# hardcamls/video-coding

Hardware: AMD Instinct MI355X
Metric: Mpixel/s decoded (1080p 4:2:0 batch) (higher is better)
Workload: dtype int32

## Files before the change

### video-coding_amd/csrc/hvc_capi.hip

```cpp
#include <cmath>

#include "hvc_ctx.h"
#include "hvc_dct_fixed.h"

bool pin_to_ctx_cpus(const hvc_ctx *c) {
    if (!c->have_cpus) {
        if (c->have_default_cpus) (void)pthread_setaffinity_np(pthread_self(), sizeof(cpu_set_t), &c->default_cpus);
        return true;
    }
    return pthread_setaffinity_np(pthread_self(), sizeof(cpu_set_t), &c->cpus) == 0;
}

bool parse_cpulist(const char *s, cpu_set_t &set) {
    CPU_ZERO(&set);
    int n = 0;
    while (*s) {
        while (*s == ' ' || *s == '\n') s++;
        if (!*s) break;
        char *end = nullptr;
        const long a = std::strtol(s, &end, 10);
        if (end == s || a < 0) return false;
        long b = a;
        s = end;
        if (*s == '-') {
// ... 147 lines not shown
    bool ok = g.ok && hipStreamCreateWithFlags(&c->own_stream, hipStreamNonBlocking) == hipSuccess &&
              hipEventCreate(&c->ev0) == hipSuccess && hipEventCreate(&c->ev1) == hipSuccess &&
              [&] {
                  for (int i = 0; i < HVC_PROF_RING; i++)
                      if (hipEventCreate(&c->k0[i]) != hipSuccess || hipEventCreate(&c->k1[i]) != hipSuccess) return false;
                  return true;
              }() &&
              hipMalloc((void **)&c->d_fix_count, HVC_FIX_WORDS * sizeof(unsigned)) == hipSuccess &&
              hipMemset(c->d_fix_count, 0, HVC_FIX_WORDS * sizeof(unsigned)) == hipSuccess;
    if (!ok) {
        hvc_destroy(c);
        return HVC_E_NO_DEVICE;
    }
    c->stream = c->own_stream;
    c->have_default_cpus = sched_getaffinity(0, sizeof c->default_cpus, &c->default_cpus) == 0;
    if (const char *env = std::getenv("HVC_HOST_CPUS")) (void)hvc_set_host_cpus(c, env);
    *out = c;
    return HVC_OK;
} HVC_ABI_CATCH

void hvc_destroy(hvc_ctx *c) {
    if (!c) return;
    c->pool.shutdown();
    DeviceGuard g(c->device);
    (void)hipStreamSynchronize(c->stream);
    if (c->own_stream) (void)hipStreamSynchronize(c->own_stream);
    if (c->copy_stream) (void)hipStreamSynchronize(c->copy_stream);
    if (c->down_stream) (void)hipStreamSynchronize(c->down_stream);
    if (c->side_stream) (void)hipStreamSynchronize(c->side_stream);
    for (int i = 0; i < 3; i++)
        if (c->rd_stream[i]) (void)hipStreamSynchronize(c->rd_stream[i]);
    if (c->d_fix_count) (void)hipFree(c->d_fix_count);
    if (c->d_fix_list) (void)hipFree(c->d_fix_list);
    if (c->d_in) (void)hipFree(c->d_in);
    if (c->d_out) (void)hipFree(c->d_out);
    if (c->d_div_px) (void)hipFree(c->d_div_px);
    if (c->d_div_in) (void)hipFree(c->d_div_in);
    if (c->d_div_out) (void)hipFree(c->d_div_out);
    if (c->d_dct_tab) (void)hipFree(c->d_dct_tab);
    if (c->d_dct_a) (void)hipFree(c->d_dct_a);
    if (c->d_dct_b) (void)hipFree(c->d_dct_b);
    if (c->d_sums) (void)hipFree(c->d_sums);
    if (c->d_aux) (void)hipFree(c->d_aux);
    if (c->d_aux2) (void)hipFree(c->d_aux2);
    if (c->ev0) (void)hipEventDestroy(c->ev0);
    if (c->ev1) (void)hipEventDestroy(c->ev1);
    for (int i = 0; i < HVC_PROF_RING; i++) {
        if (c->k0[i]) (void)hipEventDestroy(c->k0[i]);
        if (c->k1[i]) (void)hipEventDestroy(c->k1[i]);
    }
    for (int i = 0; i < hvc_ctx::RING; i++) {
        if (c->h_ring[i]) (void)hipHostFree(c->h_ring[i]);
        if (c->d_ring[i]) (void)hipFree(c->d_ring[i]);
        if (c->d_oring[i]) (void)hipFree(c->d_oring[i]);
        if (c->ev_h2d[i]) (void)hipEventDestroy(c->ev_h2d[i]);
        if (c->ev_kern[i]) (void)hipEventDestroy(c->ev_kern[i]);
        if (c->eh_in[i]) (void)hipHostFree(c->eh_in[i]);
        if (c->eh_out[i]) (void)hipHostFree(c->eh_out[i]);
        if (c->ed_in[i]) (void)hipFree(c->ed_in[i]);
        if (c->ed_out[i]) (void)hipFree(c->ed_out[i]);
        if (c->ev_up[i]) (void)hipEventDestroy(c->ev_up[i]);
        if (c->ev_down[i]) (void)hipEventDestroy(c->ev_down[i]);
        for (int k = 0; k < 3; k++)
            if (c->ev_et[i][k]) (void)hipEventDestroy(c->ev_et[i][k]);
        if (c->ev_gpu[i]) (void)hipEventDestroy(c->ev_gpu[i]);
        if (c->gp_h_ecs[i]) (void)hipHostFree(c->gp_h_ecs[i]);
// ... 269 lines not shown
    return HVC_OK;
} HVC_ABI_CATCH

int hvc_checksum_records(hvc_ctx *c, const void *data, size_t record_bytes, size_t record_stride, int n_records,
                         uint64_t *sums, int where) try {
    if (!c || !sums || n_records < 0 || (!data && n_records && record_bytes)) return HVC_E_INVALID_ARG;
    if (where != HVC_MEM_HOST && where != HVC_MEM_DEVICE) return HVC_E_INVALID_ARG;
    if (n_records == 0) return HVC_OK;
    if (n_records > 1 && record_stride < record_bytes) return HVC_E_INVALID_ARG;
    DeviceGuard g(c->device);
    if (!g.ok) return fail_hip(c, hipErrorInvalidDevice);
    const size_t sum_bytes = (size_t)n_records * sizeof(unsigned long long);
    const uint8_t *d = (const uint8_t *)data;
    int r;
    if (where == HVC_MEM_HOST) {
        const size_t bytes = (size_t)(n_records - 1) * record_stride + record_bytes;
        if ((r = grow(c, &c->d_in, &c->in_cap, bytes ? bytes : 1))) return r;
        if (bytes) HIPCHK(c, hipMemcpyAsync(c->d_in, data, bytes, hipMemcpyHostToDevice, c->stream));
        d = (const uint8_t *)c->d_in;
    }
    if ((r = grow(c, &c->d_sums, &c->sums_cap, sum_bytes))) return r;
    for (int r0 = 0; r0 < n_records; r0 += 65535)
        HIPCHK(c, hvc::launch_checksum(d + (size_t)r0 * record_stride, record_bytes, record_stride,
                                       n_records - r0 < 65535 ? n_records - r0 : 65535, (unsigned long long *)c->d_sums + r0, c->stream));
    HIPCHK(c, hipMemcpyAsync(sums, c->d_sums, sum_bytes, hipMemcpyDeviceToHost, c->stream));
    HIPCHK(c, hipStreamSynchronize(c->stream));
    return HVC_OK;
} HVC_ABI_CATCH

int hvc_last_wide_blocks(hvc_ctx *c, uint64_t *count) try {
    if (!c || !count) return HVC_E_INVALID_ARG;
    DeviceGuard g(c->device);
    unsigned long long v = 0;
    HIPCHK(c, hipMemcpyAsync(&v, c->d_fix_count + 2, sizeof v, hipMemcpyDeviceToHost, c->stream));
    HIPCHK(c, hipStreamSynchronize(c->stream));
    *count = c->wide_host >= 0 ? (uint64_t)c->wide_host : (uint64_t)v;
    return HVC_OK;
} HVC_ABI_CATCH

static void prepare_tables(const uint16_t *qtabs, int n_qtabs, int *qt, int *ethr, int *ethr_packed, unsigned *qpair) {
    for (int i = 0; i < n_qtabs * 64; i++) qt[i] = (int)qtabs[i];
    for (int t = 0; t < n_qtabs; t++) {
        unsigned qmax = 1;
        for (int i = 0; i < 64; i++) qmax = qtabs[t * 64 + i] > qmax ? qtabs[t * 64 + i] : qmax;
        unsigned long long m = HVC_GUARD_D / qmax;
        unsigned long long thr = m * m;
        ethr[t] = thr > 0x7ffffffeull ? 0x7ffffffe : (int)thr;
        m = HVC_GUARD_D_PACKED / qmax;
        thr = m * m;
        ethr_packed[t] = thr > 0x7ffffffeull ? 0x7ffffffe : (int)thr;
        static const int PAIRS[4][2] = {{HVC_PAIR_A_LO, HVC_PAIR_A_HI}, {HVC_PAIR_B_LO, HVC_PAIR_B_HI},
                                        {HVC_PAIR_C_LO, HVC_PAIR_C_HI}, {HVC_PAIR_Z_LO, HVC_PAIR_Z_HI}};
        for (int r = 0; r < 8; r++)
            for (int k = 0; k < 4; k++) {
                unsigned lo = qtabs[t * 64 + hvc::HVC_ZF[8 * r + PAIRS[k][0]]];
                unsigned hi = qtabs[t * 64 + hvc::HVC_ZF[8 * r + PAIRS[k][1]]];
                qpair[t * 32 + r * 4 + k] = (lo & 0xffffu) | (hi << 16);
            }
    }
}

static int upload_dcfix(hvc_ctx *c, const std::vector<unsigned> &ids, const std::vector<long long> &dcs, const unsigned **d_count,
                        const unsigned **d_ids, const long long **d_dcs) {
    const size_t n = ids.size();
    const size_t off_ids = 16, off_dcs = (off_ids + n * sizeof(unsigned) + 15) & ~(size_t)15;
    int r = grow(c, &c->d_dcfix, &c->dcfix_cap, off_dcs + n * sizeof(long long));
    if (r) return r;
// ... 173 lines not shown
    int per = frames_per_launch(n_frames, blocks_per_frame);
    if (per > 65535) per = 65535;
    const unsigned long long by_ids = ids_per_frame ? ((1ull << 32) - 1) / ids_per_frame : (unsigned long long)per;
    if ((unsigned long long)per > by_ids) per = (int)by_ids;
    return per < 1 ? 1 : per;
}

int decode_frames_impl(hvc_ctx *c, const int16_t *coefs, size_t coef_fs, const uint16_t *qtabs, int n_qtabs,
                       const hvc_component *comps_in, int n_comp_in, int n_frames, uint8_t *pixels, size_t pixel_fs, int where,
                       const int16_t *dc_plane, size_t dc_fs, const std::vector<WideFix> *wide) {
    if (!c || n_frames < 0) return HVC_E_INVALID_ARG;
    if (where != HVC_MEM_HOST && where != HVC_MEM_DEVICE) return HVC_E_INVALID_ARG;
    int r = check_qtabs(qtabs, n_qtabs, false);
    if (r) return r;
    hvc_component kept[HVC_MAX_COMP];
    int n_comp = 0;
    if ((r = drop_empty_components(comps_in, n_comp_in, kept, &n_comp))) return r;
    if (n_comp == 0) return HVC_OK;
    const hvc_component *const comps = kept;
    if (!coefs || !pixels) return HVC_E_INVALID_ARG;
    Layout L;
    r = make_layout(comps, n_comp, n_qtabs, L);
    if (r) return r;
    if (n_frames == 0) return HVC_OK;
    if (n_frames > 1 && (coef_fs < L.coef_span || pixel_fs < L.pixel_span)) return HVC_E_INVALID_ARG;
    if ((coef_fs & 7) || (pixel_fs & 7)) return HVC_E_ALIGNMENT;
    const unsigned long long ids_per_frame = (unsigned long long)L.tiles_per_frame * HVC_TILE;
    const int per = frames_per_launch_capped(n_frames, L.blocks_per_frame, ids_per_frame);
    if (wide && !wide->empty() && (unsigned long long)n_frames * ids_per_frame >= (1ull << 32)) return HVC_E_TOO_LARGE;
    DeviceGuard g(c->device);
    if (!g.ok) return fail_hip(c, hipErrorInvalidDevice);

    const bool twin = c->arith == HVC_ARITH_HARDCAML;
    size_t need = twin ? 0 : (size_t)((unsigned long long)per * ids_per_frame);
    if (need > c->fix_cap) {
        void *p = c->d_fix_list;
        size_t cap = c->fix_cap * sizeof(unsigned);
        r = grow(c, &p, &cap, need * sizeof(unsigned));
        c->d_fix_list = (unsigned *)p;
        c->fix_cap = cap / sizeof(unsigned);
        if (r) return r;
    }

    hvc::DecodeParams P;
    std::memset(&P, 0, sizeof P);
    P.coef_fs = coef_fs;
    P.pixel_fs = pixel_fs;
    P.n_frames = n_frames;
    P.n_comp = L.n_comp;
    P.tiles_per_frame = L.tiles_per_frame;
    for (int i = 0; i < L.n_comp; i++) P.comp[i] = L.comp[i];
    prepare_tables(qtabs, n_qtabs, P.qt, P.ethr, P.ethr_packed, P.qpair);
    wide_total_begin(c);
    fix_assign(c, P);

    bool wide_only = false;
    for (int i = 0; i < n_qtabs * 64; i++) wide_only |= qtabs[i] > 255;
    wide_only |= c->decode_kernel == 2;
    P.kernel_sel = (c->decode_kernel == 1 || c->decode_kernel == 3) ? c->decode_kernel : 0;
    if (wide_only) c->wide_host = (long long)((unsigned long long)n_frames * L.blocks_per_frame);
    if (twin) c->wide_host = 0;
    auto launch = [&](hvc::DecodeParams &Q, hipEvent_t k0, hipEvent_t k1) -> hipError_t {
        if (twin) return hvc::launch_hardcaml(hardcaml_params(Q, qtabs, n_qtabs), c->stream, k0, k1);
        if (wide_only) return hvc::launch_decode_wide_only(Q, c->stream, k0, k1);
        fix_assign(c, Q);
        const hipError_t e = hvc::launch_decode(Q, c->stream, k0, k1);
        if (e == hipSuccess) fix_commit(c);
        else fix_reset(c);
        return e;
    };
    auto launch_range = [&](const int16_t *d_coefs, uint8_t *d_pixels, int f0, int cnt, hipEvent_t k0, hipEvent_t k1) -> hipError_t {
        for (int f = f0; f < f0 + cnt; f += per) {
            hvc::DecodeParams Pk = P;
            Pk.n_frames = f0 + cnt - f < per ? f0 + cnt - f : per;
            Pk.coefs = d_coefs + (size_t)f * coef_fs;
            Pk.pixels = d_pixels + (size_t)f * pixel_fs;
            if (dc_plane) Pk.dc_plane = dc_plane + (size_t)f * dc_fs;
            const hipError_t e = launch(Pk, f == f0 ? k0 : nullptr, f + per >= f0 + cnt ? k1 : nullptr);
            if (e != hipSuccess) return e;
        }
        return hipSuccess;
    };

    if (where == HVC_MEM_DEVICE) {
        if (((uintptr_t)coefs & 15) || ((uintptr_t)pixels & 7)) return HVC_E_ALIGNMENT;
        if (dc_plane && P.kernel_sel != 0 && !twin) return HVC_E_INVALID_ARG;
        P.coefs = coefs;
        P.pixels = pixels;
        P.dc_plane = dc_plane;
        P.dc_fs = dc_fs;
        const bool prof = c->profiling;
        const int slot = (int)(c->k_calls % HVC_PROF_RING);
        HIPCHK(c, launch_range(coefs, pixels, 0, n_frames, prof ? c->k0[slot] : nullptr, prof ? c->k1[slot] : nullptr));
        if (prof) c->k_calls++;
        if (wide && !wide->empty()) return apply_wide_dc(c, P, *wide, qtabs, n_qtabs);
        return HVC_OK;
    }
    if (dc_plane || (wide && !wide->empty())) return HVC_E_INVALID_ARG;

    size_t cbytes = ((size_t)(n_frames - 1) * coef_fs + L.coef_span) * sizeof(int16_t);
    size_t pbytes = (size_t)(n_frames - 1) * pixel_fs + L.pixel_span;
// ... 217 lines not shown
    const bool aligned = width % 16 == 0 && frame_stride % 16 == 0 && (where == HVC_MEM_HOST || (uintptr_t)frames % 16 == 0);
    hvc::plan_decode_444(P, aligned);
    const unsigned long long ids_per_frame = (unsigned long long)P.tiles_per_frame * HVC_TILE * P.nw;
    const int per = frames_per_launch_capped(n_frames, L.blocks_per_frame, ids_per_frame);
    if (wide && !wide->empty() && (unsigned long long)n_frames * ids_per_frame >= (1ull << 32)) return HVC_E_TOO_LARGE;
    const unsigned long long ids = (unsigned long long)per * ids_per_frame;
    DeviceGuard g(c->device);
    if (!g.ok) return fail_hip(c, hipErrorInvalidDevice);
    if ((size_t)ids > c->fix_cap) {
        void *p = c->d_fix_list;
        size_t cap = c->fix_cap * sizeof(unsigned);
        r = grow(c, &p, &cap, (size_t)ids * sizeof(unsigned));
        c->d_fix_list = (unsigned *)p;
        c->fix_cap = cap / sizeof(unsigned);
        if (r) return r;
    }
    int ethr_unused[HVC_MAX_QTABS];
    prepare_tables(qtabs, n_qtabs, P.qt, ethr_unused, P.ethr_packed, P.qpair);
    bool wide_only = c->decode_kernel == 2;
    for (int i = 0; i < n_qtabs * 64; i++) wide_only |= qtabs[i] > 255;
    P.fix_list = c->d_fix_list;
    wide_total_begin(c);
    const int split = (aligned && !wide_only && c->decode_kernel == 0 && height % 8 == 0 && P.pl[0].cbw == P.pl[0].bw) ? fused444_mode() : 0;
    const size_t luma_ids = split ? (size_t)per * (size_t)((P.pl[0].cbw * P.pl[0].cbh + HVC_TILE - 1) / HVC_TILE) * HVC_TILE : 0;
    if (luma_ids + (size_t)ids > c->fix_cap) {
        void *p = c->d_fix_list;
        size_t cap = c->fix_cap * sizeof(unsigned);
        r = grow(c, &p, &cap, (luma_ids + (size_t)ids) * sizeof(unsigned));
        c->d_fix_list = (unsigned *)p;
        c->fix_cap = cap / sizeof(unsigned);
        if (r) return r;
        P.fix_list = c->d_fix_list;
    }
    if (split == 2 && !c->side_stream) {
        static const int prio_sel = [] { const char *v = std::getenv("HVC_444_SIDE_PRIO"); return v ? std::atoi(v) : 0; }();
        int least = 0, greatest = 0;
        HIPCHK(c, hipDeviceGetStreamPriorityRange(&least, &greatest));
        HIPCHK(c, hipStreamCreateWithPriority(&c->side_stream, hipStreamNonBlocking, prio_sel < 0 ? greatest : prio_sel > 0 ? least : 0));
        HIPCHK(c, hipEventCreateWithFlags(&c->ev_fork, hipEventDisableTiming));
        HIPCHK(c, hipEventCreateWithFlags(&c->ev_join, hipEventDisableTiming));
    }
    auto launch_split = [&](hvc::Decode444Params &Q, hipEvent_t k0, hipEvent_t k1) -> hipError_t {
        const hvc::Plane444K &K = Q.pl[0];
        hvc::DecodeParams Y;
        std::memset(&Y, 0, sizeof Y);
        Y.coefs = Q.coefs;
        Y.pixels = Q.out;
        Y.coef_fs = Q.coef_fs;
        Y.pixel_fs = Q.out_fs;
        Y.n_frames = Q.n_frames;
        Y.n_comp = 1;
        Y.comp[0].bw = K.cbw;
        Y.comp[0].bh = K.cbh;
        Y.comp[0].nblk = K.cbw * K.cbh;
        Y.comp[0].magic = K.cbw == 1 ? 0u : (unsigned)(((1ull << 32) + (unsigned)K.cbw - 1) / (unsigned)K.cbw);
        Y.comp[0].qtab = K.qtab;
        Y.comp[0].coef_off = K.coef_off;
        Y.comp[0].plane_off = K.out_off;
        Y.comp[0].stride = (size_t)Q.width;
        Y.tiles_per_frame = (Y.comp[0].nblk + HVC_TILE - 1) / HVC_TILE;
        prepare_tables(qtabs, n_qtabs, Y.qt, Y.ethr, Y.ethr_packed, Y.qpair);
        Y.dc_plane = Q.dc_plane;
        Y.dc_fs = Q.dc_fs;
        Y.fix_count = c->d_fix_count + 4 + c->fix_phase_l;
        Y.fix_count_next = c->d_fix_count + 4 + (c->fix_phase_l ^ 1);
        Y.fix_list = c->d_fix_list + (size_t)ids;
        Y.wide_total = reinterpret_cast<unsigned long long *>(c->d_fix_count + 2);
        fix_assign(c, Q);
        Q.tile0 = Q.y_tiles;
        hipStream_t ys = c->stream;
        hipError_t e = hipSuccess;
        if (k0) e = hipEventRecord(k0, c->stream);
        if (split == 2) {
            if (e == hipSuccess && !c->wide_total_started) e = hipMemsetAsync(Y.wide_total, 0, sizeof(unsigned long long), c->stream);
            Y.wide_first = Q.wide_first = 2;
            if (e == hipSuccess) e = hipEventRecord(c->ev_fork, c->stream);
            if (e == hipSuccess) e = hipStreamWaitEvent(c->side_stream, c->ev_fork, 0);
            ys = c->side_stream;
        } else {
            Y.wide_first = Q.wide_first;
            Q.wide_first = 0;
        }
        if (e == hipSuccess) e = hvc::launch_decode(Y, ys, nullptr, nullptr);
        if (e == hipSuccess) c->fix_phase_l ^= 1;
        if (e == hipSuccess) e = hvc::launch_decode_444(Q, false, c->stream, nullptr, nullptr);
        if (e == hipSuccess && split == 2) {
            e = hipEventRecord(c->ev_join, c->side_stream);
            if (e == hipSuccess) e = hipStreamWaitEvent(c->stream, c->ev_join, 0);
        }
        if (e == hipSuccess && k1) e = hipEventRecord(k1, c->stream);
        if (e == hipSuccess) fix_commit(c);
        else {
            if (c->side_stream) (void)hipStreamSynchronize(c->side_stream);
            fix_reset(c);
        }
        return e;
    };
    auto launch = [&](hvc::Decode444Params &Q, hipEvent_t k0, hipEvent_t k1) -> hipError_t {
        if (wide_only) {
            c->wide_host = (long long)n_frames * ((long long)P.pl[0].cbw * P.pl[0].cbh + 2ll * P.pl[1].cbw * P.pl[1].cbh);
            return hvc::launch_decode_444(Q, true, c->stream, k0, k1);
        }
        if (split) return launch_split(Q, k0, k1);
        fix_assign(c, Q);
        const hipError_t e = hvc::launch_decode_444(Q, false, c->stream, k0, k1);
        if (e == hipSuccess) fix_commit(c);
        else fix_reset(c);
        return e;
    };

    auto launch_range = [&](const int16_t *d_coefs, uint8_t *d_out, int f0, int cnt, hipEvent_t k0, hipEvent_t k1) -> hipError_t {
        for (int f = f0; f < f0 + cnt; f += per) {
            hvc::Decode444Params Pk = P;
            Pk.n_frames = f0 + cnt - f < per ? f0 + cnt - f : per;
            Pk.coefs = d_coefs + (size_t)f * coef_fs;
            Pk.out = d_out + (size_t)f * frame_stride;
            if (dc_plane) Pk.dc_plane = dc_plane + (size_t)f * dc_fs;
// ... 594 lines not shown
```

### video-coding_amd/csrc/hvc_ctx.h

```cpp
#ifndef HVC_CTX_H
#define HVC_CTX_H

#include <hip/hip_runtime.h>
#include <pthread.h>
#include <sched.h>

#include <algorithm>
#include <atomic>
#include <chrono>
#include <condition_variable>
#include <cstdio>
#include <cstdlib>
#include <cstring>
#include <mutex>
#include <new>
#include <thread>
#include <deque>
#include <functional>
#include <vector>

#include "../../include/hvc_jpeg.h"
#include "hvc_hdec.h"
#include "hvc_hardcaml.h"
#include "hvc_huff.h"
#include "hvc_kernels.h"
#include "hvc_pool.h"

#define HVC_PROF_RING 64
#define HVC_FIX_WORDS 8

struct hvc_ctx {
    int device = -1;
    hipStream_t own_stream = nullptr;
    hipStream_t stream = nullptr;
    hipEvent_t ev0 = nullptr, ev1 = nullptr;
    hipEvent_t k0[HVC_PROF_RING] = {}, k1[HVC_PROF_RING] = {};
    unsigned long long k_calls = 0;
    bool profiling = false;
    bool honour_restart = false;
    int decode_kernel = 0;
    int arith = HVC_ARITH_MODEL;
    int enc_arith = HVC_ARITH_MODEL;
    int huff_tables = HVC_HUFF_DEFAULT;
    int restart_interval = 0;
    unsigned *d_fix_count = nullptr;
    int fix_phase_l = 0;
    hipStream_t side_stream = nullptr;
    hipEvent_t ev_fork = nullptr, ev_join = nullptr;
    bool wide_total_started = false;
    long long wide_host = -1;
    int fix_phase = 0;
    int fix_last = 0;
    unsigned *d_fix_list = nullptr;
    size_t fix_cap = 0;
    void *d_in = nullptr, *d_out = nullptr, *d_sums = nullptr, *d_aux = nullptr, *d_aux2 = nullptr;
    size_t in_cap = 0, out_cap = 0, sums_cap = 0, aux_cap = 0, aux2_cap = 0;
    void *d_div_px = nullptr, *d_div_in = nullptr, *d_div_out = nullptr;
    size_t div_px_cap = 0, div_in_cap = 0, div_out_cap = 0;
    void *d_dct_tab = nullptr, *d_dct_a = nullptr, *d_dct_b = nullptr;
    size_t dct_a_cap = 0, dct_b_cap = 0;
    int last_hip = 0;
    static constexpr int RING = 3;
    hipStream_t copy_stream = nullptr, down_stream = nullptr;
    hipStream_t rd_stream[3] = {};
    hipEvent_t ev_rd[3] = {};
    void *h_ring[RING] = {}, *d_ring[RING] = {}, *d_oring[RING] = {};
    size_t ring_bytes = 0, oring_bytes = 0;
    hipEvent_t ev_h2d[RING] = {}, ev_kern[RING] = {}, ev_t[4] = {};
    void *eh_in[RING] = {}, *ed_in[RING] = {}, *eh_out[RING] = {}, *ed_out[RING] = {};
    size_t e_in_bytes = 0, e_out_bytes = 0;
    hipEvent_t ev_up[RING] = {}, ev_down[RING] = {}, ev_et[RING][3] = {}, ev_gpu[RING] = {};
    void *ed_seg[RING] = {}, *ed_off[RING] = {}, *eh_off[RING] = {};
    size_t e_seg_bytes = 0, e_off_bytes = 0;
    void *eh_specs[RING] = {};
    size_t e_specs_bytes = 0;
    void *gp_h_ecs[RING] = {}, *gp_d_ecs[RING] = {}, *gp_h_meta[RING] = {}, *gp_d_meta[RING] = {};
    void *gp_h_ftabs[RING] = {}, *gp_d_ftabs[RING] = {};
    size_t gp_ecs_bytes = 0, gp_meta_bytes = 0, gp_ftabs_bytes = 0;
    void *gd_ecs = nullptr, *gd_meta = nullptr, *gd_state = nullptr, *gd_tables = nullptr, *gd_coefs = nullptr, *gd_dcd = nullptr;
    void *gd_h_ecs = nullptr;
    size_t gd_h_ecs_cap = 0;
    void *gd_fcnt = nullptr;
    size_t gd_fcnt_cap = 0;
    void *gd_ftabs = nullptr;
    size_t gd_ftabs_cap = 0;
    void *gd_dcv = nullptr;
    size_t gd_dcv_cap = 0;
// ... 30 lines not shown
#endif

struct DeviceGuard {
    int prev = -1;
    bool ok = true;
    explicit DeviceGuard(int dev) {
        if (hipGetDevice(&prev) != hipSuccess) prev = -1;
        if (prev != dev) ok = hipSetDevice(dev) == hipSuccess;
    }
    ~DeviceGuard() {
        int cur = -1;
        if (prev >= 0 && hipGetDevice(&cur) == hipSuccess && cur != prev) (void)hipSetDevice(prev);
    }
};

inline int fail_hip(hvc_ctx *c, hipError_t e) {
    c->last_hip = (int)e;
    return HVC_E_HIP;
}
#define HIPCHK(c, call)                                 \
    do {                                                \
        hipError_t e_ = (call);                         \
        if (e_ != hipSuccess) return fail_hip((c), e_); \
    } while (0)

bool pin_to_ctx_cpus(const hvc_ctx *c);

inline int pool_ready(hvc_ctx *c, int n, int extra = 0) { return c->pool.ensure(n + extra); }

bool parse_cpulist(const char *s, cpu_set_t &set);

int grow(hvc_ctx *c, void **p, size_t *cap, size_t need);

template <class Params>
inline void fix_assign(const hvc_ctx *c, Params &P) {
    P.fix_count = c->d_fix_count + c->fix_phase;
    P.fix_count_next = c->d_fix_count + (c->fix_phase ^ 1);
    P.fix_list = c->d_fix_list;
    P.wide_total = reinterpret_cast<unsigned long long *>(c->d_fix_count + 2);
    P.wide_first = c->wide_total_started ? 0 : 1;
}
inline void fix_commit(hvc_ctx *c) {
    c->fix_last = c->fix_phase;
    c->fix_phase ^= 1;
    c->wide_total_started = true;
}
inline void wide_total_begin(hvc_ctx *c) {
    c->wide_total_started = false;
    c->wide_host = -1;
}
inline void fix_reset(hvc_ctx *c) {
    (void)hipMemsetAsync(c->d_fix_count, 0, HVC_FIX_WORDS * sizeof(unsigned), c->stream);
}

size_t launch_bytes_limit();
#ifndef HVC_444_MODE_DEFAULT
#define HVC_444_MODE_DEFAULT 0
#endif
int fused444_mode();
int frames_per_launch(int n_frames, unsigned long long blocks_per_frame);

struct Layout {
    hvc::CompK comp[HVC_MAX_COMP];
    int n_comp = 0, tiles_per_frame = 0;
    size_t coef_span = 0;
    size_t pixel_span = 0;
    unsigned long long blocks_per_frame = 0;
};
int make_layout(const hvc_component *comps, int n_comp, int n_qtabs, Layout &L);
int check_qtabs(const uint16_t *qtabs, int n_qtabs, bool divides);

int drop_empty_components(const hvc_component *comps, int n_comp, hvc_component *kept, int *n_kept);

struct RecordRun {
    size_t first = 0, len = 0;
};
RecordRun pixel_run(const hvc_component *comps, int n_comp);
RecordRun coef_run(const hvc_component *comps, int n_comp);
hipError_t download_pixels(const hvc_component *comps, int n_comp, const RecordRun &run, int f0, int cnt, size_t fs,
                           const uint8_t *d_base, uint8_t *h_base, hipStream_t st);
hipError_t download_coefs(const hvc_component *comps, int n_comp, const RecordRun &run, int f0, int cnt, size_t fs_bytes,
                          const uint8_t *d_base, uint8_t *h_base, hipStream_t st);

hipError_t wait_event(hipEvent_t e);

// ... 100 lines not shown
```

### video-coding_amd/csrc/hvc_kernels.h

```cpp
#ifndef HVC_KERNELS_H
#define HVC_KERNELS_H

#include <hip/hip_runtime.h>
#include <cstdlib>
#include <stddef.h>
#include <stdint.h>

#define HVC_MAX_COMP 4
#define HVC_MAX_QTABS 4
#define HVC_GUARD_D ((1 << 17) - 1)
#define HVC_TILE 256

#include "hvc_idct_spec.h"

namespace hvc {

static const unsigned char HVC_ZF[64] = {
    0,  1,  5,  6,  14, 15, 27, 28, 2,  4,  7,  13, 16, 26, 29, 42, 3,  8,  12, 17, 25, 30,
    41, 43, 9,  11, 18, 24, 31, 40, 44, 53, 10, 19, 23, 32, 39, 45, 52, 54, 20, 22, 33, 38,
    46, 51, 55, 60, 21, 34, 37, 47, 50, 56, 59, 61, 35, 36, 48, 49, 57, 58, 62, 63};

struct CompK {
    int bw, bh;
    int nblk;
    int tile0;
    unsigned magic;
    int qtab;
    size_t coef_off;
    size_t plane_off;
    size_t stride;
};

struct DecodeParams {
    const int16_t *coefs;
    uint8_t *pixels;
    size_t coef_fs;
    size_t pixel_fs;
    int n_frames, n_comp, tiles_per_frame;
    int kernel_sel;
    CompK comp[HVC_MAX_COMP];
    int qt[HVC_MAX_QTABS * 64];
    int ethr[HVC_MAX_QTABS];
    unsigned qpair[HVC_MAX_QTABS * 32];
    int ethr_packed[HVC_MAX_QTABS];
    unsigned *fix_count;
    unsigned *fix_count_next;
    unsigned *fix_list;
    const int16_t *dc_plane;
    size_t dc_fs;
    unsigned long long *wide_total;
    int wide_first;
    int xcd_map;
    unsigned xcd_magic;
};

struct EncodeParams {
    const uint8_t *pixels;
    int16_t *coefs;
    size_t coef_fs, pixel_fs;
    int n_frames, n_comp, tiles_per_frame, xcd_map;
    unsigned xcd_magic, pad;
    CompK comp[HVC_MAX_COMP];
    float qrcp[HVC_MAX_QTABS * 64];
};

struct UpsampleParams {
    const uint8_t *src;
    uint8_t *dst;
    int cw, ch, n_planes, xcd_map;
    size_t src_stride, dst_stride, src_ps, dst_ps;
    unsigned xcd_magic, pad;
};

struct Plane444K {
    int bw;
    int cbw, cbh;
    int aw, ah;
    int qtab;
    size_t coef_off;
    size_t out_off;
};

#define HVC_444_TILE_BW 64
// ... 31 lines not shown
    static const int run444 = [] { const char *v = getenv("HVC_XCD_RUN_444"); return v ? atoi(v) : -1; }();
    if (fused) return run444 >= 0 ? run444 : run >= 0 ? run : 64;
    return run >= 0 ? run : 16;
}
#ifdef __HIPCC__
__device__ __forceinline__ void xcd_work(int map, unsigned magic, unsigned &frame, unsigned &tile) {
    frame = blockIdx.y;
    tile = blockIdx.x;
    if (map > 0) {
        const unsigned per = gridDim.x, id = frame * per + tile, sh = (unsigned)map - 1u;
        const unsigned group = 8u << sh, total = per * gridDim.y;
        if (id < total - total % group) {
            const unsigned k = id >> 3;
            const unsigned lin = ((((k >> sh) << 3) + (id & 7u)) << sh) + (k & ((1u << sh) - 1u));
            frame = __umulhi(lin, magic);
            tile = lin - frame * per;
        }
    }
}
#endif
inline int xcd_map_for(unsigned per, unsigned n, unsigned &magic, bool fused = false) {
    magic = per > 1 ? (unsigned)(((1ull << 32) + per - 1) / per) : 0u;
    const int run = xcd_map_run(fused);
    if (run <= 0 || per <= 1 || (unsigned long long)per * n * per >= (1ull << 32)) return 0;
    int sh = 0;
    while ((1 << (sh + 1)) <= run) sh++;
    return sh + 1;
}

hipError_t launch_decode_444(const Decode444Params &P, bool wide_only, hipStream_t s, hipEvent_t k0 = nullptr,
                             hipEvent_t k1 = nullptr);
void plan_decode_444(Decode444Params &P, bool aligned);
hipError_t launch_decode(const DecodeParams &P, hipStream_t s, hipEvent_t k0 = nullptr, hipEvent_t k1 = nullptr);
hipError_t launch_decode_wide_only(const DecodeParams &P, hipStream_t s, hipEvent_t k0 = nullptr, hipEvent_t k1 = nullptr);
hipError_t launch_decode_dcfix(const DecodeParams &P, const unsigned *count, const unsigned *ids, const long long *dcs,
                               hipStream_t s);
hipError_t launch_decode_444_dcfix(const Decode444Params &P, const unsigned *count, const unsigned *ids, const long long *dcs,
                                   unsigned n_host, hipStream_t s);
hipError_t launch_encode(const EncodeParams &P, hipStream_t s, hipEvent_t k0 = nullptr, hipEvent_t k1 = nullptr);
hipError_t launch_upsample420(const UpsampleParams &P, hipStream_t s);
hipError_t launch_abs_error(const EncodeParams &P, const uint8_t *recon, uint8_t *error, hipStream_t s);
#define HVC_CHECKSUM_MUL 0x9E3779B97F4A7C15ull
hipError_t launch_checksum(const uint8_t *data, size_t record_bytes, size_t record_stride, int n_records,
                           unsigned long long *sums, hipStream_t s);

}
#endif
```

### video-coding_amd/csrc/hvc_kernels.hip

```cpp

#include <hip/hip_runtime.h>
#include <stdint.h>
#include <stdlib.h>
#include <string.h>

#include "hvc_idct_spec.h"
#include "hvc_kernels.h"

#ifndef HVC_FAST_LB
#define HVC_FAST_LB HVC_TILE
#endif

namespace hvc {

__device__ constexpr int ZI[64] = {
    0,  1,  8,  16, 9,  2,  3,  10, 17, 24, 32, 25, 18, 11, 4,  5,
    12, 19, 26, 33, 40, 48, 41, 34, 27, 20, 13, 6,  7,  14, 21, 28,
    35, 42, 49, 56, 57, 50, 43, 36, 29, 22, 15, 23, 30, 37, 44, 51,
    58, 59, 52, 45, 38, 31, 39, 46, 53, 60, 61, 54, 47, 55, 62, 63};
__device__ constexpr int ZF[64] = {
    0,  1,  5,  6,  14, 15, 27, 28, 2,  4,  7,  13, 16, 26, 29, 42,
    3,  8,  12, 17, 25, 30, 41, 43, 9,  11, 18, 24, 31, 40, 44, 53,
    10, 19, 23, 32, 39, 45, 52, 54, 20, 22, 33, 38, 46, 51, 55, 60,
    21, 34, 37, 47, 50, 56, 59, 61, 35, 36, 48, 49, 57, 58, 62, 63};
// ... 403 lines not shown
__global__ __launch_bounds__(HVC_PACKED_LB) void k_decode_packed(DecodeParams P) {
    BlockRef br;
    const int lane = threadIdx.x;
    unsigned wframe, wtile;
    xcd_work(P.xcd_map, P.xcd_magic, wframe, wtile);
    const bool active = locate(P, (int)wframe, (int)wtile, lane, br);
    const uint4 *src = reinterpret_cast<const uint4 *>(P.coefs + br.coef_idx);
    const unsigned *__restrict__ qp = P.qpair + br.qtab * 32;
    PackedGuard g;
    unsigned out[8][2];
    int16_t dcv = 0;
    if (DCP) dcv = P.dc_plane[(size_t)wframe * P.dc_fs + ((br.coef_idx - (size_t)wframe * P.coef_fs) >> 6)];
#if HVC_TRAFFIC_ONLY == 2
    const bool hvc_full = __ballot(active) == ~0ull;
    const int hvc_src_stride = hvc_full ? 64 : 1;
    if (hvc_full) src = src - 8 * (lane & 63) + (lane & 63);
#endif
    HVC_DECODE_BLOCK_PACKED(src, qp, out, g, if (DCP) w[0] = with_dc(w[0], dcv););
#ifdef HVC_K1_PAD_VALU
    {
        int pad = lane;
#pragma unroll
        for (int i = 0; i < HVC_K1_PAD_VALU; i++) asm volatile("v_mul_i32_i24 %0, %0, %1" : "+v"(pad) : "v"(lane));
        asm volatile("" ::"v"(pad));
    }
#endif

    const bool bad = packed_guard_failed(g, P.ethr_packed[br.qtab]);
    if (active && !bad) {
#pragma unroll
        for (int j = 0; j < 8; j++)
            store_row8(P.pixels + br.pix_idx + (size_t)j * br.stride, out[j][0], out[j][1]);
    }
    const bool flag = active && bad;
    const unsigned long long m = __ballot(flag);
    if (m) {
        const int wl = lane & 63;
        unsigned base = 0;
        if (wl == 0) base = atomicAdd(P.fix_count, (unsigned)__popcll(m));
        base = __shfl(base, 0);
        if (flag) {
            unsigned idx = base + (unsigned)__popcll(m & ((1ull << wl) - 1ull));
            P.fix_list[idx] = (wframe * (unsigned)P.tiles_per_frame + wtile) * HVC_TILE + lane;
        }
    }
}

constexpr int Q16_ITERS = HVC_TILE / 16;

__device__ __forceinline__ int dot2vv(unsigned pair, unsigned k, int add) {
    int d;
    asm("v_dot2_i32_i16 %0, %1, %2, %3" : "=v"(d) : "v"(pair), "v"(k), "v"(add));
    return d;
}
__device__ __forceinline__ int partner(int v) { return __builtin_amdgcn_mov_dpp(v, 0xB1, 0xf, 0xf, true); }

struct Q16Lane {
    unsigned k00, k01, k10, k11;
    int a0, a1, sh0, sh1;
};

__device__ __forceinline__ void q16_pass(unsigned P0, unsigned P1, const Q16Lane &K, bool odd, int negm, int (&o)[4],
                                         int &ymax, int &ymin) {
    const int p = dot2vv(P0, K.k00, K.a0) >> K.sh0, q = dot2vv(P0, K.k01, K.a0) >> K.sh0;
    const int s = dot2vv(P1, K.k10, K.a1) >> K.sh1, t = dot2vv(P1, K.k11, K.a1) >> K.sh1;
    const int u1 = p + s, u2 = p - s, u3 = q + t, u4 = q - t;
    const int ys = odd ? u2 + u4 : 0, yd = odd ? u2 - u4 : 0;
    ymax = max(max(ymax, ys), yd);
    ymin = min(min(ymin, ys), yd);
    const int w2 = mad24(181, ys, 128) >> 8, w4 = mad24(181, yd, 128) >> 8;
    const int m0 = u1, m1 = odd ? u3 : u2, m2 = odd ? w2 : u3, m3 = odd ? w4 : u4;
    o[0] = partner(m0) + ((m0 ^ negm) - negm);
    o[1] = partner(m1) + ((m1 ^ negm) - negm);
    o[2] = partner(m2) + ((m2 ^ negm) - negm);
    o[3] = partner(m3) + ((m3 ^ negm) - negm);
}

// ... 183 lines not shown
#endif
__global__ __launch_bounds__(HVC_FIXUP_LANES) void k_decode_wide(DecodeParams P, const unsigned *count, const unsigned *list,
                                                                 const long long *dc_list) {
    const unsigned long long n = (unsigned long long)*count;
    if (blockIdx.x == 0 && threadIdx.x == 0) {
        if (P.fix_count_next) *P.fix_count_next = 0;
        if (P.wide_total) {
            if (P.wide_first == 2) atomicAdd(P.wide_total, n);
            else *P.wide_total = P.wide_first ? n : *P.wide_total + n;
        }
    }
    for (unsigned long long i = (unsigned long long)blockIdx.x * blockDim.x + threadIdx.x; i < n;
         i += (unsigned long long)gridDim.x * blockDim.x) {
        const unsigned long long id = list[i];
        const int lane = (int)(id % HVC_TILE);
        const unsigned long long t = id / HVC_TILE;
        const int tile = (int)(t % (unsigned)P.tiles_per_frame);
        const int frame = (int)(t / (unsigned)P.tiles_per_frame);
        if (frame >= P.n_frames) continue;
        BlockRef br;
        if (!locate(P, frame, tile, lane, br)) continue;
        unsigned w[32], out[8][2];
        load_block_dwords(P.coefs + br.coef_idx, w);
        int64_t dc = 0;
        if (P.dc_plane)
            dc = (int64_t)P.dc_plane[(size_t)frame * P.dc_fs + ((br.coef_idx - (size_t)frame * P.coef_fs) >> 6)];
        if (dc_list) dc = (int64_t)dc_list[i];
        decode_block_wide<true>(w, P.qt + br.qtab * 64, P.dc_plane != nullptr || dc_list != nullptr, dc, out);
#pragma unroll
        for (int j = 0; j < 8; j++) store_row8(P.pixels + br.pix_idx + (size_t)j * br.stride, out[j][0], out[j][1]);
    }
}

__global__ __launch_bounds__(HVC_TILE) void k_decode_wide_all(DecodeParams P) {
    BlockRef br;
    const int lane = threadIdx.x;
    unsigned wframe, wtile;
    xcd_work(P.xcd_map, P.xcd_magic, wframe, wtile);
    const bool active = locate(P, (int)wframe, (int)wtile, lane, br);
    unsigned w[32], out[8][2];
    load_block_dwords(P.coefs + br.coef_idx, w);
    int64_t dc = 0;
    if (P.dc_plane) dc = (int64_t)P.dc_plane[(size_t)wframe * P.dc_fs + ((br.coef_idx - (size_t)wframe * P.coef_fs) >> 6)];
    decode_block_wide<false>(w, P.qt + br.qtab * 64, P.dc_plane != nullptr, dc, out);
    if (active) {
#pragma unroll
        for (int j = 0; j < 8; j++) store_row8(P.pixels + br.pix_idx + (size_t)j * br.stride, out[j][0], out[j][1]);
    }
}

struct Ref444 {
    int p, bx, by;
    bool active;
    bool store;
};

__device__ __forceinline__ Ref444 locate444(const Decode444Params &P, int tile, int lane, int wgs, int tw) {
    Ref444 r;
    if (tile < P.y_tiles) {
        const Plane444K &K = P.pl[0];
        const int n = K.cbw * K.cbh;
        int b = tile * wgs + lane;
        r.active = b < n;
        b = r.active ? b : n - 1;
        const unsigned by = K.cbw == 1 ? (unsigned)b : __umulhi((unsigned)b, P.y_magic);
        r.p = 0;
// ... 633 lines not shown
            s1 += (unsigned)k * b;
        }
        acc += (2ull * (16ull * v) + 1ull) * s0 + 2ull * s1;
    }
    if (blockIdx.x == 0)
        for (size_t i = vec * 16 + threadIdx.x; i < record_bytes; i += 256) acc += (2ull * i + 1ull) * ((unsigned long long)rec[i] + 1ull);
    acc *= HVC_CHECKSUM_MUL;
#pragma unroll
    for (int o = 32; o > 0; o >>= 1) acc += __shfl_xor(acc, o);
    if ((threadIdx.x & 63) == 0 && acc) atomicAdd(&sums[blockIdx.y], acc);
}

hipError_t launch_checksum(const uint8_t *data, size_t record_bytes, size_t record_stride, int n_records,
                           unsigned long long *sums, hipStream_t s) {
    if (n_records <= 0) return hipSuccess;
    hipError_t e = hipMemsetAsync(sums, 0, (size_t)n_records * sizeof(unsigned long long), s);
    if (e != hipSuccess) return e;
    if (record_bytes == 0) return hipSuccess;
    const size_t pieces = (record_bytes / 16 + 255) / 256;
    size_t gx = pieces < 1 ? 1 : pieces;
    const size_t want = (size_t)(4096 + n_records - 1) / (size_t)n_records;
    if (gx > want) gx = want;
    hipLaunchKernelGGL(k_checksum, dim3((unsigned)gx, (unsigned)n_records, 1), dim3(256), 0, s, data, record_bytes,
                       record_stride, sums);
    return hipGetLastError();
}


hipError_t launch_decode(const DecodeParams &P, hipStream_t s, hipEvent_t k0, hipEvent_t k1) {
    if (P.n_frames <= 0 || P.tiles_per_frame <= 0) return hipSuccess;
    hipError_t e;
    dim3 grid((unsigned)P.tiles_per_frame, (unsigned)P.n_frames, 1);
    if (k0 && (e = hipEventRecord(k0, s)) != hipSuccess) return e;
    static const int env_sel = [] {
        const char *v = getenv("HVC_DECODE_KERNEL");
        return !v ? 0 : (v[0] == 'v' && v[1] == '2') ? 1 : (v[0] == 'q') ? 3 : 0;
    }();
    const int sel = P.kernel_sel ? P.kernel_sel : P.dc_plane ? 0 : env_sel;
    if (P.dc_plane && sel != 0) return hipErrorInvalidValue;
    if (sel == 3)
        hipLaunchKernelGGL(k_decode_q16, grid, dim3(HVC_TILE), 0, s, P);
    else if (sel == 1)
        hipLaunchKernelGGL(k_decode_fast, grid, dim3(HVC_TILE), 0, s, P);
    else {
        static const unsigned pad = [] { const char *v = getenv("HVC_DEC_LDS_PAD"); return v ? (unsigned)atoi(v) : 0u; }();
        DecodeParams Q = P;
        Q.xcd_map = xcd_map_for(grid.x, grid.y, Q.xcd_magic);
        if (P.dc_plane)
            hipLaunchKernelGGL(k_decode_packed<true>, grid, dim3(HVC_TILE), pad, s, Q);
        else
            hipLaunchKernelGGL(k_decode_packed<false>, grid, dim3(HVC_TILE), pad, s, Q);
    }
    e = hipGetLastError();
    if (e != hipSuccess) return e;
    if (k1 && (e = hipEventRecord(k1, s)) != hipSuccess) return e;
    hipLaunchKernelGGL(k_decode_wide, dim3(HVC_FIXUP_WGS), dim3(HVC_FIXUP_LANES), 0, s, P, P.fix_count, P.fix_list, (const long long *)nullptr);
    return hipGetLastError();
}

hipError_t launch_decode_dcfix(const DecodeParams &P, const unsigned *count, const unsigned *ids, const long long *dcs,
                               hipStream_t s) {
    DecodeParams Q = P;
    Q.fix_count_next = nullptr;
    Q.wide_total = nullptr;
    hipLaunchKernelGGL(k_decode_wide, dim3(64), dim3(64), 0, s, Q, count, ids, dcs);
    return hipGetLastError();
}

hipError_t launch_decode_444_dcfix(const Decode444Params &P, const unsigned *count, const unsigned *ids, const long long *dcs,
                                   unsigned n_host, hipStream_t s) {
    Decode444Params Q = P;
    Q.fix_count_next = nullptr;
    Q.wide_total = nullptr;
    hipLaunchKernelGGL(k_decode_wide_444, dim3(64), dim3(64), 0, s, Q, count, ids, 0ull, dcs);
    const size_t W = (size_t)P.width;
    const bool aligned = (W % 16 == 0) && (P.out_fs % 16 == 0) && ((uintptr_t)P.out % 16 == 0);
    const long long hw = aligned ? P.pl[1].aw / 8 : P.pl[1].aw;
    const long long seams = 2 * (long long)(P.c_tiles_y - 1) * hw;
    const long long want = seams > (long long)n_host * 81 ? seams : (long long)n_host * 81;
    const dim3 rgrid((unsigned)((want + 255) / 256) ? (unsigned)((want + 255) / 256) : 1u, (unsigned)P.n_frames, 1);
    if (aligned)
        hipLaunchKernelGGL(k_reinterp_444<true>, rgrid, dim3(256), 0, s, Q, count, ids, 0);
    else
        hipLaunchKernelGGL(k_reinterp_444<false>, rgrid, dim3(256), 0, s, Q, count, ids, 0);
    return hipGetLastError();
}

hipError_t launch_decode_wide_only(const DecodeParams &P, hipStream_t s, hipEvent_t k0, hipEvent_t k1) {
    if (P.n_frames <= 0 || P.tiles_per_frame <= 0) return hipSuccess;
    hipError_t e;
// ... 116 lines not shown
```

Baseline: 1.348 million.

## Replace atomic fixup list with per-wave ballot masks in packed decode

The packed decode kernel stops appending overflow block ids to a global list through atomicAdd and instead writes each wave's ballot mask into a per-tile mask array, plus a sequence flag marking that some block needs the wide path. A new fixup kernel returns early when the flag does not match, and otherwise scans the mask words in segmented order, clears them, and re-decodes the flagged blocks on the wide path. The wide-total counter now alternates between two slots, so the next one is zeroed inside the kernel rather than through a separate memset. This removes global atomics and the list writes from the hot kernel and makes the fixup close to free when nothing overflows, at the cost of a full mask scan when any block does, extra buffer management, and more complex bookkeeping for the 4:4:4 split path.

```diff
diff --git a/video-coding_amd/csrc/hvc_capi.hip b/video-coding_amd/csrc/hvc_capi.hip
--- a/video-coding_amd/csrc/hvc_capi.hip
+++ b/video-coding_amd/csrc/hvc_capi.hip
@@ -203,6 +203,7 @@
         if (c->rd_stream[i]) (void)hipStreamSynchronize(c->rd_stream[i]);
     if (c->d_fix_count) (void)hipFree(c->d_fix_count);
     if (c->d_fix_list) (void)hipFree(c->d_fix_list);
+    if (c->d_fix_masks) (void)hipFree(c->d_fix_masks);
     if (c->d_in) (void)hipFree(c->d_in);
     if (c->d_out) (void)hipFree(c->d_out);
     if (c->d_div_px) (void)hipFree(c->d_div_px);
@@ -538,7 +539,7 @@
     if (!c || !count) return HVC_E_INVALID_ARG;
     DeviceGuard g(c->device);
     unsigned long long v = 0;
-    HIPCHK(c, hipMemcpyAsync(&v, c->d_fix_count + 2, sizeof v, hipMemcpyDeviceToHost, c->stream));
+    HIPCHK(c, hipMemcpyAsync(&v, wide_total_ptr(c, c->total_slot), sizeof v, hipMemcpyDeviceToHost, c->stream));
     HIPCHK(c, hipStreamSynchronize(c->stream));
     *count = c->wide_host >= 0 ? (uint64_t)c->wide_host : (uint64_t)v;
     return HVC_OK;
@@ -778,7 +779,14 @@
     if (!g.ok) return fail_hip(c, hipErrorInvalidDevice);
 
     const bool twin = c->arith == HVC_ARITH_HARDCAML;
-    size_t need = twin ? 0 : (size_t)((unsigned long long)per * ids_per_frame);
+    bool wide_only = false;
+    for (int i = 0; i < n_qtabs * 64; i++) wide_only |= qtabs[i] > 255;
+    wide_only |= c->decode_kernel == 2;
+    const int kernel_sel = (c->decode_kernel == 1 || c->decode_kernel == 3) ? c->decode_kernel : 0;
+    const bool block_stage = !twin && !wide_only;
+    const bool uses_list = block_stage && (kernel_sel != 0 || hvc::decode_kernel_env() != 0);
+    if (block_stage && (r = fix_masks_reserve(c, per < n_frames ? per : n_frames, L.tiles_per_frame))) return r;
+    size_t need = uses_list ? (size_t)((unsigned long long)per * ids_per_frame) : 0;
     if (need > c->fix_cap) {
         void *p = c->d_fix_list;
         size_t cap = c->fix_cap * sizeof(unsigned);
@@ -800,19 +808,20 @@
     wide_total_begin(c);
     fix_assign(c, P);
 
-    bool wide_only = false;
-    for (int i = 0; i < n_qtabs * 64; i++) wide_only |= qtabs[i] > 255;
-    wide_only |= c->decode_kernel == 2;
-    P.kernel_sel = (c->decode_kernel == 1 || c->decode_kernel == 3) ? c->decode_kernel : 0;
+    P.kernel_sel = kernel_sel;
     if (wide_only) c->wide_host = (long long)((unsigned long long)n_frames * L.blocks_per_frame);
     if (twin) c->wide_host = 0;
     auto launch = [&](hvc::DecodeParams &Q, hipEvent_t k0, hipEvent_t k1) -> hipError_t {
         if (twin) return hvc::launch_hardcaml(hardcaml_params(Q, qtabs, n_qtabs), c->stream, k0, k1);
         if (wide_only) return hvc::launch_decode_wide_only(Q, c->stream, k0, k1);
         fix_assign(c, Q);
-        const hipError_t e = hvc::launch_decode(Q, c->stream, k0, k1);
-        if (e == hipSuccess) fix_commit(c);
-        else fix_reset(c);
+        const bool packed = hvc::decode_kernel_for(Q) == 0;
+        hipError_t e = packed ? masks_assign(c, Q, c->stream) : hipSuccess;
+        if (e == hipSuccess) e = hvc::launch_decode(Q, c->stream, k0, k1);
+        if (e == hipSuccess) {
+            fix_commit(c, !packed);
+            if (packed) masks_commit(c, Q);
+        } else fix_reset(c);
         return e;
     };
     auto launch_range = [&](const int16_t *d_coefs, uint8_t *d_pixels, int f0, int cnt, hipEvent_t k0, hipEvent_t k1) -> hipError_t {
@@ -1096,6 +1105,7 @@
         if (r) return r;
         P.fix_list = c->d_fix_list;
     }
+    if (split && (r = fix_masks_reserve(c, per < n_frames ? per : n_frames, (P.pl[0].cbw * P.pl[0].cbh + HVC_TILE - 1) / HVC_TILE))) return r;
     if (split == 2 && !c->side_stream) {
         static const int prio_sel = [] { const char *v = std::getenv("HVC_444_SIDE_PRIO"); return v ? std::atoi(v) : 0; }();
         int least = 0, greatest = 0;
@@ -1129,8 +1139,8 @@
         Y.fix_count = c->d_fix_count + 4 + c->fix_phase_l;
         Y.fix_count_next = c->d_fix_count + 4 + (c->fix_phase_l ^ 1);
         Y.fix_list = c->d_fix_list + (size_t)ids;
-        Y.wide_total = reinterpret_cast<unsigned long long *>(c->d_fix_count + 2);
         fix_assign(c, Q);
+        Y.wide_total = Q.wide_total;
         Q.tile0 = Q.y_tiles;
         hipStream_t ys = c->stream;
         hipError_t e = hipSuccess;
@@ -1145,8 +1155,14 @@
             Y.wide_first = Q.wide_first;
             Q.wide_first = 0;
         }
+        const bool packed = hvc::decode_kernel_for(Y) == 0;
+        if (e == hipSuccess && packed) {
+            e = masks_assign(c, Y, c->stream);
+            Q.wide_total = Y.wide_total;
+        }
         if (e == hipSuccess) e = hvc::launch_decode(Y, ys, nullptr, nullptr);
-        if (e == hipSuccess) c->fix_phase_l ^= 1;
+        if (e == hipSuccess && packed) masks_commit(c, Y);
+        if (e == hipSuccess && !packed) c->fix_phase_l ^= 1;
         if (e == hipSuccess) e = hvc::launch_decode_444(Q, false, c->stream, nullptr, nullptr);
         if (e == hipSuccess && split == 2) {
             e = hipEventRecord(c->ev_join, c->side_stream);
diff --git a/video-coding_amd/csrc/hvc_ctx.h b/video-coding_amd/csrc/hvc_ctx.h
--- a/video-coding_amd/csrc/hvc_ctx.h
+++ b/video-coding_amd/csrc/hvc_ctx.h
@@ -27,7 +27,7 @@
 #include "hvc_pool.h"
 
 #define HVC_PROF_RING 64
-#define HVC_FIX_WORDS 8
+#define HVC_FIX_WORDS 10
 
 struct hvc_ctx {
     int device = -1;
@@ -53,6 +53,10 @@
     int fix_last = 0;
     unsigned *d_fix_list = nullptr;
     size_t fix_cap = 0;
+    void *d_fix_masks = nullptr;
+    size_t fix_masks_cap = 0;
+    int total_slot = 0, total_zero = -1;
+    unsigned long long masks_seq = 0;
     void *d_in = nullptr, *d_out = nullptr, *d_sums = nullptr, *d_aux = nullptr, *d_aux2 = nullptr;
     size_t in_cap = 0, out_cap = 0, sums_cap = 0, aux_cap = 0, aux2_cap = 0;
     void *d_div_px = nullptr, *d_div_in = nullptr, *d_div_out = nullptr;
@@ -149,25 +153,57 @@
 
 int grow(hvc_ctx *c, void **p, size_t *cap, size_t need);
 
+inline unsigned long long *wide_total_ptr(const hvc_ctx *c, int slot) {
+    return reinterpret_cast<unsigned long long *>(c->d_fix_count + (slot ? 6 : 2));
+}
 template <class Params>
 inline void fix_assign(const hvc_ctx *c, Params &P) {
     P.fix_count = c->d_fix_count + c->fix_phase;
     P.fix_count_next = c->d_fix_count + (c->fix_phase ^ 1);
     P.fix_list = c->d_fix_list;
-    P.wide_total = reinterpret_cast<unsigned long long *>(c->d_fix_count + 2);
+    P.wide_total = wide_total_ptr(c, c->total_slot);
     P.wide_first = c->wide_total_started ? 0 : 1;
 }
-inline void fix_commit(hvc_ctx *c) {
-    c->fix_last = c->fix_phase;
-    c->fix_phase ^= 1;
+inline hipError_t masks_assign(hvc_ctx *c, hvc::DecodeParams &P, hipStream_t stream) {
+    P.fix_masks = (unsigned long long *)c->d_fix_masks;
+    P.fix_any = reinterpret_cast<unsigned long long *>(c->d_fix_count + 8);
+    P.fix_seq = ++c->masks_seq;
+    P.wide_total_next = nullptr;
+    if (P.wide_first != 1) return hipSuccess;
+    hipError_t e = hipSuccess;
+    if (c->total_zero >= 0) c->total_slot = c->total_zero;
+    else e = hipMemsetAsync(wide_total_ptr(c, c->total_slot), 0, sizeof(unsigned long long), stream);
+    c->total_zero = -1;
+    P.wide_total = wide_total_ptr(c, c->total_slot);
+    P.wide_total_next = wide_total_ptr(c, c->total_slot ^ 1);
+    return e;
+}
+inline void masks_commit(hvc_ctx *c, const hvc::DecodeParams &P) {
+    if (P.wide_total_next) c->total_zero = c->total_slot ^ 1;
+}
+inline void fix_commit(hvc_ctx *c, bool used_counters = true) {
+    if (used_counters) {
+        c->fix_last = c->fix_phase;
+        c->fix_phase ^= 1;
+    }
     c->wide_total_started = true;
 }
 inline void wide_total_begin(hvc_ctx *c) {
     c->wide_total_started = false;
     c->wide_host = -1;
 }
+inline int fix_masks_reserve(hvc_ctx *c, int frames, int tiles_per_frame) {
+    const size_t need = (size_t)hvc::decode_mask_words(frames, tiles_per_frame) * sizeof(unsigned long long);
+    if (need <= c->fix_masks_cap) return HVC_OK;
+    const int r = grow(c, &c->d_fix_masks, &c->fix_masks_cap, need);
+    if (r) return r;
+    HIPCHK(c, hipMemsetAsync(c->d_fix_masks, 0, c->fix_masks_cap, c->stream));
+    return HVC_OK;
+}
 inline void fix_reset(hvc_ctx *c) {
     (void)hipMemsetAsync(c->d_fix_count, 0, HVC_FIX_WORDS * sizeof(unsigned), c->stream);
+    c->total_zero = -1;
+    if (c->d_fix_masks) (void)hipMemsetAsync(c->d_fix_masks, 0, c->fix_masks_cap, c->stream);
 }
 
 size_t launch_bytes_limit();
diff --git a/video-coding_amd/csrc/hvc_kernels.h b/video-coding_amd/csrc/hvc_kernels.h
--- a/video-coding_amd/csrc/hvc_kernels.h
+++ b/video-coding_amd/csrc/hvc_kernels.h
@@ -46,9 +46,13 @@
     unsigned *fix_count;
     unsigned *fix_count_next;
     unsigned *fix_list;
+    unsigned long long *fix_masks;
+    unsigned long long *fix_any;
+    unsigned long long fix_seq;
     const int16_t *dc_plane;
     size_t dc_fs;
     unsigned long long *wide_total;
+    unsigned long long *wide_total_next;
     int wide_first;
     int xcd_map;
     unsigned xcd_magic;
@@ -146,6 +150,11 @@
                              hipEvent_t k1 = nullptr);
 void plan_decode_444(Decode444Params &P, bool aligned);
 hipError_t launch_decode(const DecodeParams &P, hipStream_t s, hipEvent_t k0 = nullptr, hipEvent_t k1 = nullptr);
+inline unsigned long long decode_mask_words(int n_frames, int tiles_per_frame) {
+    return (unsigned long long)n_frames * (unsigned long long)tiles_per_frame * (HVC_TILE / 64);
+}
+int decode_kernel_env();
+inline int decode_kernel_for(const DecodeParams &P) { return P.kernel_sel ? P.kernel_sel : P.dc_plane ? 0 : decode_kernel_env(); }
 hipError_t launch_decode_wide_only(const DecodeParams &P, hipStream_t s, hipEvent_t k0 = nullptr, hipEvent_t k1 = nullptr);
 hipError_t launch_decode_dcfix(const DecodeParams &P, const unsigned *count, const unsigned *ids, const long long *dcs,
                                hipStream_t s);
diff --git a/video-coding_amd/csrc/hvc_kernels.hip b/video-coding_amd/csrc/hvc_kernels.hip
--- a/video-coding_amd/csrc/hvc_kernels.hip
+++ b/video-coding_amd/csrc/hvc_kernels.hip
@@ -459,17 +459,10 @@
         for (int j = 0; j < 8; j++)
             store_row8(P.pixels + br.pix_idx + (size_t)j * br.stride, out[j][0], out[j][1]);
     }
-    const bool flag = active && bad;
-    const unsigned long long m = __ballot(flag);
-    if (m) {
-        const int wl = lane & 63;
-        unsigned base = 0;
-        if (wl == 0) base = atomicAdd(P.fix_count, (unsigned)__popcll(m));
-        base = __shfl(base, 0);
-        if (flag) {
-            unsigned idx = base + (unsigned)__popcll(m & ((1ull << wl) - 1ull));
-            P.fix_list[idx] = (wframe * (unsigned)P.tiles_per_frame + wtile) * HVC_TILE + lane;
-        }
+    const unsigned long long m = __ballot(active && bad);
+    if (m && (lane & 63) == 0) {
+        P.fix_masks[(wframe * (unsigned)P.tiles_per_frame + wtile) * (HVC_TILE / 64) + ((unsigned)lane >> 6)] = m;
+        *P.fix_any = P.fix_seq;
     }
 }
 
@@ -719,6 +712,73 @@
     }
 }
 
+#define HVC_FIXUP_UNROLL 4
+__global__ __launch_bounds__(HVC_FIXUP_LANES) void k_decode_wide_masks(DecodeParams P, unsigned long long *masks,
+                                                                       unsigned long long n_words, int seg_shift) {
+    const unsigned wl = threadIdx.x & 63u;
+    if (P.wide_total_next && blockIdx.x == 0 && threadIdx.x == 0) *P.wide_total_next = 0;
+    if (*P.fix_any != P.fix_seq) return;
+    const unsigned long long waves = (unsigned long long)gridDim.x * (HVC_FIXUP_LANES / 64);
+    const unsigned long long wave = __builtin_amdgcn_readfirstlane(blockIdx.x * (HVC_FIXUP_LANES / 64) + (threadIdx.x >> 6));
+    const unsigned seg_mask = (1u << seg_shift) - 1u;
+    unsigned long long seen = 0;
+    auto word_of = [&](unsigned long long round, unsigned v) {
+        const unsigned long long seg = (round * (64 * HVC_FIXUP_UNROLL) + v) >> seg_shift;
+        return ((seg * waves + wave) << seg_shift) + (v & seg_mask);
+    };
+    for (unsigned long long round = 0; word_of(round, 0) < n_words; round++) {
+        unsigned long long mw[HVC_FIXUP_UNROLL], nz[HVC_FIXUP_UNROLL];
+#pragma unroll
+        for (int k = 0; k < HVC_FIXUP_UNROLL; k++) {
+            const unsigned long long idx = word_of(round, 64u * k + wl);
+            mw[k] = idx < n_words ? masks[idx] : 0ull;
+            if (mw[k] != 0ull) masks[idx] = 0ull;
+        }
+#pragma unroll
+        for (int k = 0; k < HVC_FIXUP_UNROLL; k++) nz[k] = __ballot(mw[k] != 0ull);
+        for (;;) {
+            unsigned long long cur = 0;
+            unsigned v = 0;
+            bool found = false;
+#pragma unroll
+            for (int k = 0; k < HVC_FIXUP_UNROLL; k++)
+                if (!found && nz[k]) {
+                    v = 64u * k + (unsigned)(__ffsll((long long)nz[k]) - 1);
+                    nz[k] &= nz[k] - 1;
+                    cur = mw[k];
+                    found = true;
+                }
+            if (!found) break;
+            const unsigned src = v & 63u;
+            const unsigned long long m = (unsigned long long)(unsigned)__builtin_amdgcn_readlane((int)(unsigned)cur, src) |
+                                         (unsigned long long)(unsigned)__builtin_amdgcn_readlane((int)(unsigned)(cur >> 32), src) << 32;
+            const unsigned long long word = word_of(round, v);
+            const unsigned long long t = word / (HVC_TILE / 64);
+            const unsigned long long frame = t / (unsigned)P.tiles_per_frame;
+            if (frame >= (unsigned long long)P.n_frames) continue;
+            const int tile = (int)(t - frame * (unsigned)P.tiles_per_frame);
+            const int lane = (int)((word % (HVC_TILE / 64)) * 64 + wl);
+            seen += (unsigned long long)__popcll(m);
+            BlockRef br;
+            if (!((m >> wl) & 1ull) || !locate(P, (int)frame, tile, lane, br)) continue;
+            unsigned w[32], out[8][2];
+            load_block_dwords(P.coefs + br.coef_idx, w);
+            int64_t dc = 0;
+            if (P.dc_plane)
+                dc = (int64_t)P.dc_plane[(size_t)frame * P.dc_fs + ((br.coef_idx - (size_t)frame * P.coef_fs) >> 6)];
+            decode_block_wide<false>(w, P.qt + br.qtab * 64, P.dc_plane != nullptr, dc, out);
+#pragma unroll
+            for (int j = 0; j < 8; j++) store_row8(P.pixels + br.pix_idx + (size_t)j * br.stride, out[j][0], out[j][1]);
+        }
+    }
+    if (wl == 0 && seen && P.wide_total) atomicAdd(P.wide_total, seen);
+}
+inline int fixup_seg_shift(unsigned long long n_words, unsigned long long waves) {
+    int sh = 0;
+    while (sh < 6 && (n_words >> (sh + 1)) >= waves * 4) sh++;
+    return sh;
+}
+
 __global__ __launch_bounds__(HVC_TILE) void k_decode_wide_all(DecodeParams P) {
     BlockRef br;
     const int lane = threadIdx.x;
@@ -1418,18 +1478,17 @@
     hipError_t e;
     dim3 grid((unsigned)P.tiles_per_frame, (unsigned)P.n_frames, 1);
     if (k0 && (e = hipEventRecord(k0, s)) != hipSuccess) return e;
-    static const int env_sel = [] {
-        const char *v = getenv("HVC_DECODE_KERNEL");
-        return !v ? 0 : (v[0] == 'v' && v[1] == '2') ? 1 : (v[0] == 'q') ? 3 : 0;
-    }();
-    const int sel = P.kernel_sel ? P.kernel_sel : P.dc_plane ? 0 : env_sel;
+    const int sel = decode_kernel_for(P);
     if (P.dc_plane && sel != 0) return hipErrorInvalidValue;
-    if (sel == 3)
-        hipLaunchKernelGGL(k_decode_q16, grid, dim3(HVC_TILE), 0, s, P);
-    else if (sel == 1)
-        hipLaunchKernelGGL(k_decode_fast, grid, dim3(HVC_TILE), 0, s, P);
-    else {
+    if (sel == 1 || sel == 3) {
+        if (!P.fix_count || !P.fix_list) return hipErrorInvalidValue;
+        if (sel == 3)
+            hipLaunchKernelGGL(k_decode_q16, grid, dim3(HVC_TILE), 0, s, P);
+        else
+            hipLaunchKernelGGL(k_decode_fast, grid, dim3(HVC_TILE), 0, s, P);
+    } else {
         static const unsigned pad = [] { const char *v = getenv("HVC_DEC_LDS_PAD"); return v ? (unsigned)atoi(v) : 0u; }();
+        if (!P.fix_masks || !P.fix_any) return hipErrorInvalidValue;
         DecodeParams Q = P;
         Q.xcd_map = xcd_map_for(grid.x, grid.y, Q.xcd_magic);
         if (P.dc_plane)
@@ -1440,8 +1499,22 @@
     e = hipGetLastError();
     if (e != hipSuccess) return e;
     if (k1 && (e = hipEventRecord(k1, s)) != hipSuccess) return e;
-    hipLaunchKernelGGL(k_decode_wide, dim3(HVC_FIXUP_WGS), dim3(HVC_FIXUP_LANES), 0, s, P, P.fix_count, P.fix_list, (const long long *)nullptr);
+    if (sel == 1 || sel == 3)
+        hipLaunchKernelGGL(k_decode_wide, dim3(HVC_FIXUP_WGS), dim3(HVC_FIXUP_LANES), 0, s, P, P.fix_count, P.fix_list, (const long long *)nullptr);
+    else {
+        const unsigned long long n_words = decode_mask_words(P.n_frames, P.tiles_per_frame);
+        const int seg_shift = fixup_seg_shift(n_words, (unsigned long long)HVC_FIXUP_WGS * (HVC_FIXUP_LANES / 64));
+        hipLaunchKernelGGL(k_decode_wide_masks, dim3(HVC_FIXUP_WGS), dim3(HVC_FIXUP_LANES), 0, s, P, P.fix_masks, n_words, seg_shift);
+    }
     return hipGetLastError();
+}
+
+int decode_kernel_env() {
+    static const int env_sel = [] {
+        const char *v = getenv("HVC_DECODE_KERNEL");
+        return !v ? 0 : (v[0] == 'v' && v[1] == '2') ? 1 : (v[0] == 'q') ? 3 : 0;
+    }();
+    return env_sel;
 }
 
 hipError_t launch_decode_dcfix(const DecodeParams &P, const unsigned *count, const unsigned *ids, const long long *dcs,
```

Measured after the change: 1.335 million. No clear change (-0.9%).
